# 18281818221/kalle-audio

Measured on AMD Instinct MI355X. Metric: audio-seconds/sec (node) DiT train step, 10s@12.5Hz x1024 latents, higher is better.
Workload: dtype bf16; 1 GPU; DiT train step (fwd+bwd+allreduce+Adam), 24 blocks D=1536 h=24, 10 s @ 12.5 Hz x 1024 latents (T=125+1 prepend), S=130 x 768 cross-attn cond; DiT shape chosen by this build (reference defines none); global_batch=256, per_gpu_batch=256, parallelism=dp1, objective=v, io_channels=1024, global_cond_type=prepend

## Files before the change

kalle_audio_amd/csrc/gemm2.hip:

```cpp
#include <stdio.h>
#include <stdlib.h>
#include <string.h>

#include <algorithm>
#include <functional>
#include <type_traits>
#include <utility>

#include "gemm_common.h"
#include "../../include/kalle_hip.h"

namespace {

constexpr int BK2 = 64;
#define GPTR(p) ((const __attribute__((address_space(1))) void*)(p))

__device__ __attribute__((aligned(64))) const unsigned kalle_zero_block[16] = {0, 0, 0, 0, 0, 0, 0, 0, 0, 0, 0, 0, 0, 0, 0, 0};

template <bool KM, int R, int NW>
struct Loader {
    static constexpr int PER_WAVE = (R / 8) / NW;
    const bf16_t* src[PER_WAVE];
    int64_t kstep;

    __device__ __forceinline__ void init(const bf16_t* X, int64_t ld, int Rtot, int r0, int k0, int wave, int lane,
                                         int glu_inner = 0, int glu_tn = 0) {
#pragma unroll
        for (int i = 0; i < PER_WAVE; ++i) {
            const int q = wave * PER_WAVE + i;
            if constexpr (!KM) {
                const int row = 8 * q + (lane >> 3);
                const int slot = lane & 7;
                const int c = slot ^ ((row >> 1) & 7);
                int gr = min(r0 + row, Rtot - 1);
                if (glu_inner > 0) {
                    const int wn_ = row >> 6, w_ = row & 63;
                    gr = (w_ >= 32 ? glu_inner : 0) + glu_tn * (R / 2) + wn_ * 32 + (w_ & 31);
                }
                src[i] = X + (int64_t)gr * ld + k0 + 8 * c;
            } else {
                constexpr int RB = 2 * R;
                constexpr int ROWS = 1024 / RB;
                const int pos = q * ROWS + (lane * 16) / RB;
                const int slot = ((lane * 16) % RB) / 16;
                const int c = slot ^ (2 * (pos & 7));
                const int krow = (pos & ~7) | ((pos & 7) ^ (((pos >> 3) & 1) << 2));
                const int gc = min(r0 + 8 * c, Rtot - 8);
                src[i] = X + (int64_t)(k0 + krow) * ld + gc;
            }
        }
        kstep = KM ? 64 * ld : 64;
    }
    __device__ __forceinline__ void issue(char* region, int wave) {
#pragma unroll
        for (int i = 0; i < PER_WAVE; ++i) {
            __builtin_amdgcn_global_load_lds(GPTR(src[i]), LDS_PTR(void, region + (wave * PER_WAVE + i) * 1024), 16, 0, 0);
            src[i] += kstep;
        }
    }
    __device__ __forceinline__ void issue_tail(char* region, int wave, int lane, int kvalid) {
#pragma unroll
        for (int i = 0; i < PER_WAVE; ++i) {
            const int q = wave * PER_WAVE + i;
            bool ok;
            if constexpr (!KM) {
                const int row = 8 * q + (lane >> 3);
                const int c = (lane & 7) ^ ((row >> 1) & 7);
                ok = 8 * c < kvalid;
            } else {
                constexpr int RB = 2 * R, ROWS = 1024 / RB;
                const int pos = q * ROWS + (lane * 16) / RB;
                const int krow = (pos & ~7) | ((pos & 7) ^ (((pos >> 3) & 1) << 2));
                ok = krow < kvalid;
            }
            const bf16_t* sp = ok ? src[i] : reinterpret_cast<const bf16_t*>(kalle_zero_block);
            __builtin_amdgcn_global_load_lds(GPTR(sp), LDS_PTR(void, region + (wave * PER_WAVE + i) * 1024), 16, 0, 0);
            src[i] += kstep;
        }
    }
    __device__ __forceinline__ void issue_at(char* region, int wave, int lane, int t, int tail_t, int kvalid) {
        if (t == tail_t) issue_tail(region, wave, lane, kvalid);
        else issue(region, wave);
    }
};

template <int OFF>
__device__ __forceinline__ i32x4 lds_b128(unsigned a) {
    i32x4 r;
    asm volatile("ds_read_b128 %0, %1 offset:%2" : "=v"(r) : "v"(a), "n"(OFF));
    return r;
}
__device__ __forceinline__ i32x2 lds_tr(unsigned a) {
    i32x2 r;
    asm volatile("ds_read_b64_tr_b16 %0, %1" : "=v"(r) : "v"(a));
    return r;
}

template <bool KM, int R>
struct Reader {
    unsigned b0[2], b1[2];
    __device__ __forceinline__ void init(int region_off, int rbase, int lane) {
#pragma unroll
        for (int s = 0; s < 2; ++s) {
            if constexpr (!KM) {
                const int row = rbase + (lane & 15);
                const int c = 4 * s + (lane >> 4);
                b0[s] = region_off + row * 128 + ((c ^ ((row >> 1) & 7)) << 4);
                b1[s] = 0;
            } else {
                constexpr int RB = 2 * R;
                const int g = lane >> 4, i = lane & 15;
                const int q = i >> 2, pp = i & 3;
                const int b = 4 * s + g;
                const int odd = b & 1;
                const int pos1 = 8 * b + (odd ? 4 : 0) + q;
                const int pos2 = 8 * b + (odd ? 0 : 4) + q;
                const int cl = (rbase >> 3) + (pp >> 1);
                const int hb = (pp & 1) * 8;
                b0[s] = region_off + pos1 * RB + ((cl ^ (2 * (pos1 & 7))) << 4) + hb;
                b1[s] = region_off + pos2 * RB + ((cl ^ (2 * (pos2 & 7))) << 4) + hb;
            }
        }
    }
    template <int S, int NTILE, int T0 = 0>
    __device__ __forceinline__ void read(unsigned so, i32x4 (&f)[NTILE]) const {
        if constexpr (!KM) {
            const unsigned a = b0[S] + so;
            f[0] = lds_b128<2048 * (T0 + 0)>(a);
            f[1] = lds_b128<2048 * (T0 + 1)>(a);
            f[2] = lds_b128<2048 * (T0 + 2)>(a);
            f[3] = lds_b128<2048 * (T0 + 3)>(a);
            if constexpr (NTILE == 8) {
                f[4] = lds_b128<2048 * (T0 + 4)>(a);
                f[5] = lds_b128<2048 * (T0 + 5)>(a);
                f[6] = lds_b128<2048 * (T0 + 6)>(a);
                f[7] = lds_b128<2048 * (T0 + 7)>(a);
            }
        } else {
            const unsigned a0 = b0[S] + so, a1 = b1[S] + so;
#pragma unroll
            for (int t = 0; t < NTILE; ++t) {
                const i32x2 lo = lds_tr(a0 ^ ((T0 + t) << 5));
                const i32x2 hi = lds_tr(a1 ^ ((T0 + t) << 5));
                f[t] = i32x4{lo[0], lo[1], hi[0], hi[1]};
            }
        }
    }
};

__device__ __forceinline__ void gemm_stamp(const GemmParams& p, int wave, int lane, int idx, int slot = -1) {
    if (p.stamps && (wave == 0 || wave == 7) && lane == 0)
        p.stamps[((int64_t)(slot < 0 ? (int)blockIdx.x : slot) * 2 + (wave ? 1 : 0)) * 8 + idx] = __builtin_amdgcn_s_memrealtime();
}

constexpr int EPI_DEPTH = 1;

struct NoHook { __device__ __forceinline__ void operator()() const {} };

__device__ __forceinline__ int pidx(int r, int c) { return r * 64 + (c ^ ((r & 1) << 2)); }

template <bool C_F32, int TM, int GLU = 0, typename Hook = NoHook>
__device__ __forceinline__ void wave_epilogue(const GemmParams& p, f32x4 (&acc)[TM][4], char* patch_base, int wave, int lane,
                                              int row0, int col0, Hook after_barrier = Hook{}, int stamp_slot = -1) {
    constexpr int DEPTH = EPI_DEPTH < TM ? EPI_DEPTH : TM;
    float* patch = reinterpret_cast<float*>(patch_base) + wave * (16 * 64);
    const int g = lane >> 4, li = lane & 15;
    const bool pre_res = C_F32 && GLU == 0 && !p.atomic && p.residual != nullptr;
    f32x4 rbuf[DEPTH][4];
    auto load_res = [&](int mt, f32x4 (&rv)[4]) {
#pragma unroll
        for (int i = 0; i < 4; ++i) {
            const int gm = row0 + 16 * mt + g + 4 * i, gn = col0 + 4 * li;
            rv[i] = f32x4{0.f, 0.f, 0.f, 0.f};
            if (gm < p.M && gn < p.N) rv[i] = *reinterpret_cast<const f32x4*>(p.residual + gemm_crow(p, gm) * p.ldr + gn);
        }
    };
    i32x4 hbuf[DEPTH][2][2];
    auto load_h = [&](int mt, i32x4 (&hv)[2][2]) {
        const int c8 = (lane & 7) * 8, j0 = col0 + c8;
#pragma unroll
        for (int half = 0; half < 2; ++half) {
            const int gm = row0 + 16 * mt + (lane >> 3) + 8 * half;
            hv[half][0] = i32x4{0, 0, 0, 0};
            hv[half][1] = i32x4{0, 0, 0, 0};
            if (gm < p.M && j0 < p.glu_inner) {
                const bf16_t* hp = static_cast<const bf16_t*>(p.glu_aux) + (int64_t)gm * 2 * p.glu_inner;
                hv[half][0] = *reinterpret_cast<const i32x4*>(hp + j0);
                hv[half][1] = *reinterpret_cast<const i32x4*>(hp + p.glu_inner + j0);
            }
        }
    };
    asm volatile("s_waitcnt lgkmcnt(0)" ::: "memory");
    __builtin_amdgcn_s_barrier();
    after_barrier();
    gemm_stamp(p, wave, lane, 3, stamp_slot);
#pragma unroll
    for (int d = 0; d < DEPTH; ++d) {
        if constexpr (GLU == 2) load_h(d, hbuf[d]);
        if (pre_res) load_res(d, rbuf[d]);
    }
    float sx[8], sg[8];
#pragma unroll
    for (int e = 0; e < 8; ++e) { sx[e] = 0.f; sg[e] = 0.f; }
    f32x4 bias4 = f32x4{0.f, 0.f, 0.f, 0.f}, bias8[2] = {f32x4{0.f, 0.f, 0.f, 0.f}, f32x4{0.f, 0.f, 0.f, 0.f}};
    float bx[8], bg[8];
#pragma unroll
    for (int e = 0; e < 8; ++e) { bx[e] = 0.f; bg[e] = 0.f; }
    if (p.bias) {
        if constexpr (GLU == 1) {
            const int j0 = col0 + (lane & 3) * 8;
            if (j0 < p.glu_inner) {
#pragma unroll
                for (int e = 0; e < 8; ++e) { bx[e] = p.bias[j0 + e]; bg[e] = p.bias[p.glu_inner + j0 + e]; }
            }
        } else if constexpr (GLU == 0) {
            if constexpr (C_F32) {
                if (!p.atomic && col0 + 4 * li < p.N) bias4 = *reinterpret_cast<const f32x4*>(p.bias + col0 + 4 * li);
            } else {
                const int gn = col0 + 8 * (lane & 7);
                if (gn < p.N) {
                    bias8[0] = *reinterpret_cast<const f32x4*>(p.bias + gn);
                    bias8[1] = *reinterpret_cast<const f32x4*>(p.bias + gn + 4);
                }
            }
        }
    }
#pragma unroll
    for (int mt = 0; mt < TM; ++mt) {
        const int slot = mt % DEPTH;
        f32x4 rcur[4];
        i32x4 hcur[2][2];
        if constexpr (GLU == 2) {
#pragma unroll
            for (int half = 0; half < 2; ++half) { hcur[half][0] = hbuf[slot][half][0]; hcur[half][1] = hbuf[slot][half][1]; }
            if (mt + DEPTH < TM) load_h(mt + DEPTH, hbuf[slot]);
        }
        if (pre_res) {
#pragma unroll
            for (int i = 0; i < 4; ++i) rcur[i] = rbuf[slot][i];
            if (mt + DEPTH < TM) load_res(mt + DEPTH, rbuf[slot]);
        }
#pragma unroll
        for (int nt = 0; nt < 4; ++nt)
#pragma unroll
            for (int r = 0; r < 4; ++r) patch[pidx(4 * g + r, 16 * nt + li)] = acc[mt][nt][r];
        asm volatile("s_waitcnt lgkmcnt(0)" ::: "memory");
        const int rbase = row0 + 16 * mt;
        if constexpr (GLU == 1) {
            const int r = lane >> 2, c8 = (lane & 3) * 8;
            const int gm = rbase + r, j0 = col0 + c8;
            if (gm < p.M && j0 < p.glu_inner) {
                float xv[8], gv[8];
#pragma unroll
                for (int e = 0; e < 8; ++e) { xv[e] = patch[pidx(r, c8 + e)]; gv[e] = patch[pidx(r, 32 + c8 + e)]; }
#pragma unroll
                for (int e = 0; e < 8; ++e) { xv[e] += bx[e]; gv[e] += bg[e]; }
                i32x4 hx, hg, av;
#pragma unroll
                for (int e = 0; e < 4; ++e) {
                    hx[e] = (int)pack_bf16x2(xv[2 * e], xv[2 * e + 1]);
                    hg[e] = (int)pack_bf16x2(gv[2 * e], gv[2 * e + 1]);
                    const float x0 = bf16lo((uint32_t)hx[e]), x1 = bf16hi((uint32_t)hx[e]);
                    const float g0 = bf16lo((uint32_t)hg[e]), g1 = bf16hi((uint32_t)hg[e]);
                    av[e] = (int)pack_bf16x2(x0 * siluf_(g0), x1 * siluf_(g1));
                }
                bf16_t* hp = reinterpret_cast<bf16_t*>(p.C) + (int64_t)gm * p.ldc;
                *reinterpret_cast<i32x4*>(hp + j0) = hx;
                *reinterpret_cast<i32x4*>(hp + p.glu_inner + j0) = hg;
                *reinterpret_cast<i32x4*>(static_cast<bf16_t*>(p.glu_aux) + (int64_t)gm * p.glu_inner + j0) = av;
            }
        } else if constexpr (GLU == 2) {
            const int c8 = (lane & 7) * 8, j0 = col0 + c8;
#pragma unroll
            for (int half = 0; half < 2; ++half) {
                const int r = (lane >> 3) + 8 * half;
                const int gm = rbase + r;
                if (gm < p.M && j0 < p.glu_inner) {
                    const i32x4 xv = hcur[half][0], gv = hcur[half][1];
                    i32x4 ox, og;
#pragma unroll
                    for (int e = 0; e < 4; ++e) {
                        const float x[2] = {bf16lo((uint32_t)xv[e]), bf16hi((uint32_t)xv[e])};
                        const float gg[2] = {bf16lo((uint32_t)gv[e]), bf16hi((uint32_t)gv[e])};
                        const float d[2] = {bf16_to_f32(f32_to_bf16(patch[pidx(r, c8 + 2 * e)] * p.alpha)),
                                            bf16_to_f32(f32_to_bf16(patch[pidx(r, c8 + 2 * e + 1)] * p.alpha))};
                        float dx[2], dg[2];
#pragma unroll
                        for (int q = 0; q < 2; ++q) {
                            const float sgm = sigmoidf_(gg[q]);
                            dx[q] = d[q] * gg[q] * sgm;
                            dg[q] = d[q] * x[q] * sgm * (1.f + gg[q] * (1.f - sgm));
                        }
                        ox[e] = (int)pack_bf16x2(dx[0], dx[1]);
                        og[e] = (int)pack_bf16x2(dg[0], dg[1]);
                        sx[2 * e] += bf16lo((uint32_t)ox[e]); sx[2 * e + 1] += bf16hi((uint32_t)ox[e]);
                        sg[2 * e] += bf16lo((uint32_t)og[e]); sg[2 * e + 1] += bf16hi((uint32_t)og[e]);
                    }
                    bf16_t* dp = reinterpret_cast<bf16_t*>(p.C) + (int64_t)gm * p.ldc;
                    *reinterpret_cast<i32x4*>(dp + j0) = ox;
                    *reinterpret_cast<i32x4*>(dp + p.glu_inner + j0) = og;
                }
            }
        } else if (p.atomic) {
            const int gn = col0 + lane;
#pragma unroll 4
            for (int r = 0; r < 16; ++r) {
                const int gm = rbase + r;
                if (gm < p.M && gn < p.N)
                    atomicAdd(reinterpret_cast<float*>(p.C) + (int64_t)gm * p.ldc + gn, patch[pidx(r, lane)] * p.alpha);
            }
        } else if constexpr (C_F32) {
#pragma unroll
            for (int i = 0; i < 4; ++i) {
                const int r = g + 4 * i;
                const int gm = rbase + r, gn = col0 + 4 * li;
                if (gm >= p.M || gn >= p.N) continue;
                const f32x4 pv = *reinterpret_cast<const f32x4*>(patch + pidx(r, 4 * li));
                float v[4] = {pv[0], pv[1], pv[2], pv[3]};
                const int64_t crow = gemm_crow(p, gm);
                gemm_epilogue4(p, gm, gn, crow, v, false, &bias4);
                if (pre_res) {
#pragma unroll
                    for (int j = 0; j < 4; ++j) v[j] += rcur[i][j];
                }
                float* cp = reinterpret_cast<float*>(p.C) + crow * p.ldc + gn;
                if (p.accumulate) {
                    const f32x4 c0 = *reinterpret_cast<const f32x4*>(cp);
#pragma unroll
                    for (int j = 0; j < 4; ++j) v[j] += c0[j];
                }
                *reinterpret_cast<f32x4*>(cp) = f32x4{v[0], v[1], v[2], v[3]};
            }
        } else {
#pragma unroll
            for (int half = 0; half < 2; ++half) {
                const int r = (lane >> 3) + 8 * half;
                const int gm = rbase + r, gn = col0 + 8 * (lane & 7);
                if (gm >= p.M || gn >= p.N) continue;
                const f32x4 p0 = *reinterpret_cast<const f32x4*>(patch + pidx(r, 8 * (lane & 7)));
                const f32x4 p1 = *reinterpret_cast<const f32x4*>(patch + pidx(r, 8 * (lane & 7) + 4));
                float v0[4] = {p0[0], p0[1], p0[2], p0[3]}, v1[4] = {p1[0], p1[1], p1[2], p1[3]};
                const int64_t crow = gemm_crow(p, gm);
                gemm_epilogue4(p, gm, gn, crow, v0, true, &bias8[0]);
                gemm_epilogue4(p, gm, gn + 4, crow, v1, true, &bias8[1]);
                i32x4 o;
                o[0] = (int)pack_bf16x2(v0[0], v0[1]);
                o[1] = (int)pack_bf16x2(v0[2], v0[3]);
                o[2] = (int)pack_bf16x2(v1[0], v1[1]);
                o[3] = (int)pack_bf16x2(v1[2], v1[3]);
                *reinterpret_cast<i32x4*>(reinterpret_cast<bf16_t*>(p.C) + crow * p.ldc + gn) = o;
            }
        }
        asm volatile("s_waitcnt lgkmcnt(0)" ::: "memory");
    }
    if constexpr (GLU == 2) {
        if (p.glu_dbias) {
#pragma unroll
            for (int e = 0; e < 8; ++e) {
#pragma unroll
                for (int o = 8; o < 64; o <<= 1) { sx[e] += __shfl_xor(sx[e], o, 64); sg[e] += __shfl_xor(sg[e], o, 64); }
            }
            const int j0 = col0 + (lane & 7) * 8;
            if (lane < 8 && j0 < p.glu_inner) {
#pragma unroll
                for (int e = 0; e < 8; ++e) {
                    atomicAdd(p.glu_dbias + j0 + e, sx[e]);
                    atomicAdd(p.glu_dbias + p.glu_inner + j0 + e, sg[e]);
                }
            }
        }
    }
    if (p.stamps) {
        gemm_stamp(p, wave, lane, 4, stamp_slot);
        asm volatile("s_waitcnt vmcnt(0)" ::: "memory");
        gemm_stamp(p, wave, lane, 5, stamp_slot);
    }
}

#define MFMA16(FA, FB)                                                                                         \
    _Pragma("unroll") for (int mt = 0; mt < 4; ++mt) _Pragma("unroll") for (int nt = 0; nt < 4; ++nt)          \
        acc[mt][nt] = __builtin_amdgcn_mfma_f32_16x16x32_bf16(__builtin_bit_cast(bf16x8, FA[mt]),              \
                                                              __builtin_bit_cast(bf16x8, FB[nt]), acc[mt][nt], 0, 0, 0)

template <bool A_KM, bool B_KM, bool C_F32, int WM, int WN, int TM, int GLU = 0, int NS = 3>
__global__ __launch_bounds__(WM * WN * 64, 2) void gemm2_kernel(GemmParams p) {
    static_assert(TM == 4, "wave tile is 64 x 64");
    constexpr int TN = 4;
    constexpr int NW = WM * WN;
    constexpr int BM = WM * TM * 16, BN = WN * TN * 16;
    constexpr int A_BYTES = BM * 128, B_BYTES = BN * 128, STAGE = A_BYTES + B_BYTES;
    extern __shared__ __attribute__((aligned(16))) char smem[];
    const unsigned lds0 = (unsigned)(size_t)LDS_PTR(char, smem);

    const int tid = threadIdx.x, lane = tid & 63;
    const int wave = __builtin_amdgcn_readfirstlane(tid >> 6);
    const int wm = wave / WN, wn = wave % WN;

    int tm, tn;
    gemm_tile_coords(blockIdx.x, gridDim.x, p.tiles_m, p.tiles_n, p.group_m, tm, tn);
    const int m0 = tm * BM, n0 = tn * BN;

    const int nk_all = (p.K + BK2 - 1) / BK2;
    const int kt0 = blockIdx.y * p.ktiles_per_split;
    const int nk = min(p.ktiles_per_split, nk_all - kt0);
    const int kvalid = p.K % BK2;
    const int tail_t = kvalid ? nk_all - 1 - kt0 : -1;

    f32x4 acc[TM][TN];
#pragma unroll
    for (int i = 0; i < TM; ++i)
#pragma unroll
        for (int j = 0; j < TN; ++j) acc[i][j] = f32x4{0.f, 0.f, 0.f, 0.f};

    Loader<A_KM, BM, NW> la;
    Loader<B_KM, BN, NW> lb;
    la.init(p.A, p.lda, p.M, m0, kt0 * BK2, wave, lane);
    lb.init(p.B, p.ldb, p.N, n0, kt0 * BK2, wave, lane, GLU == 1 ? p.glu_inner : 0, tn);
    const int arow = wm * TM * 16, bcol = wn * TN * 16;
    Reader<A_KM, BM> ra;
    Reader<B_KM, BN> rb;
    ra.init(lds0, arow, lane);
    rb.init(lds0 + A_BYTES, bcol, lane);

    {
    constexpr int PT = Loader<A_KM, BM, NW>::PER_WAVE + Loader<B_KM, BN, NW>::PER_WAVE;
    static_assert((NS - 2) * PT <= 63, "vmcnt is a 6-bit counter");
    {
        const int pre = nk < NS ? nk : NS;
#pragma unroll
        for (int t = 0; t < NS; ++t) {
            if (t < pre) {
                la.issue_at(smem + t * STAGE, wave, lane, t, tail_t, kvalid);
                lb.issue_at(smem + t * STAGE + A_BYTES, wave, lane, t, tail_t, kvalid);
            }
        }
        constexpr int PRE_KEEP = (NS - 1) * PT <= 63 ? NS - 1 : NS - 2;
        const int keep = pre - 1 < PRE_KEEP ? pre - 1 : PRE_KEEP;
        auto wait_keep = [&](auto self, auto c) {
            constexpr int C = decltype(c)::value;
            if (keep == C) asm volatile("s_waitcnt vmcnt(%0)" ::"n"(C * PT) : "memory");
            if constexpr (C > 0) self(self, std::integral_constant<int, C - 1>{});
        };
        wait_keep(wait_keep, std::integral_constant<int, PRE_KEEP>{});
    }
    __builtin_amdgcn_s_barrier();
    __builtin_amdgcn_sched_barrier(0);

    i32x4 fa0[4], fb0[4], fa1[4], fb1[4];
    ra.template read<0, 4>(0, fa0);
    rb.template read<0, 4>(0, fb0);

    unsigned so_cur = 0, so_nxt = STAGE;
    int kt = 0;

    auto iteration = [&](auto issue_c, auto next_c, auto keep_c) {
        constexpr bool ISSUE = decltype(issue_c)::value, NEXT = decltype(next_c)::value;
        constexpr int KEEP = decltype(keep_c)::value;
        asm volatile("s_waitcnt lgkmcnt(0)" ::: "memory");
        __builtin_amdgcn_sched_barrier(0);
        ra.template read<1, 4>(so_cur, fa1);
        rb.template read<1, 4>(so_cur, fb1);
        __builtin_amdgcn_sched_barrier(0);
        MFMA16(fa0, fb0);
        __builtin_amdgcn_sched_barrier(0);
        asm volatile("s_waitcnt vmcnt(%0) lgkmcnt(0)" ::"n"(KEEP * PT) : "memory");
        __builtin_amdgcn_s_barrier();
        __builtin_amdgcn_sched_barrier(0);
        if (wave >= NW / 2) {
            MFMA16(fa1, fb1);
            __builtin_amdgcn_sched_barrier(0);
        }
        if constexpr (ISSUE) {
            la.issue_at(smem + so_cur, wave, lane, kt + NS, tail_t, kvalid);
            lb.issue_at(smem + so_cur + A_BYTES, wave, lane, kt + NS, tail_t, kvalid);
        }
        if constexpr (NEXT) {
            ra.template read<0, 4>(so_nxt, fa0);
            rb.template read<0, 4>(so_nxt, fb0);
        }
        __builtin_amdgcn_sched_barrier(0);
        if (wave < NW / 2) {
            MFMA16(fa1, fb1);
            __builtin_amdgcn_sched_barrier(0);
        }
        so_cur = so_nxt;
        so_nxt = so_nxt + STAGE >= NS * STAGE ? 0 : so_nxt + STAGE;
    };
    using T_ = std::true_type;
    using F_ = std::false_type;
#pragma unroll 1
    for (; kt + NS < nk; ++kt) iteration(T_{}, T_{}, std::integral_constant<int, NS - 2>{});
    auto tail = [&](auto self, auto r) {
        constexpr int R = decltype(r)::value;
        if (nk - 1 - kt == R) { iteration(F_{}, T_{}, std::integral_constant<int, R - 1>{}); ++kt; }
        if constexpr (R > 1) self(self, std::integral_constant<int, R - 1>{});
    };
    tail(tail, std::integral_constant<int, NS - 1>{});
    iteration(F_{}, F_{}, std::integral_constant<int, 0>{});
    }

    if constexpr (C_F32) {
        if (p.slab_stride) {
            GemmParams q = p;
            q.C = static_cast<float*>(p.C) + (int64_t)blockIdx.y * p.slab_stride;
            wave_epilogue<C_F32, TM>(q, acc, smem, wave, lane, m0 + arow, n0 + bcol);
            return;
        }
    }
    wave_epilogue<C_F32, TM, GLU>(p, acc, smem, wave, lane, m0 + arow, GLU == 1 ? tn * (BN / 2) + wn * 32 : n0 + bcol);
}


template <bool B_KM, bool C_F32, int WM, int WN, int GLU, int NS>
__global__ __launch_bounds__(WM * WN * 128, 1) void gemm2_ks2_kernel(GemmParams p) {
    static_assert(!B_KM || WN >= 2, "a k-major operand tile needs >= 128 columns (16 swizzle slots per k-row)");
    constexpr int TM = 4, TN = 4;
    constexpr int NWT = WM * WN, NW = 2 * NWT;
    constexpr int BM = WM * 64, BN = WN * 64;
    constexpr int A_BYTES = BM * 128, B_BYTES = BN * 128, STAGE = A_BYTES + B_BYTES;
    constexpr int RED_OFF = 32768;
    static_assert(RED_OFF + NWT * 16384 <= NS * STAGE, "partial-sum exchange must fit into the ring");
    extern __shared__ __attribute__((aligned(16))) char smem[];
    const unsigned lds0 = (unsigned)(size_t)LDS_PTR(char, smem);

    const int tid = threadIdx.x, lane = tid & 63;
    const int wave = __builtin_amdgcn_readfirstlane(tid >> 6);
    const int kg = wave / NWT, wt = wave % NWT;
    const int wm = wt / WN, wn = wt % WN;

// ... 180 lines not shown
__device__ __forceinline__ int sched_resolve(int xcd, int raw, int first_round, int ntiles) {
    const int id = xcd + 8 * (first_round + raw);
    return id < ntiles ? id : ntiles;
}
__device__ __forceinline__ void sched_leave(int* sched, int nwg) {
    if (atomicAdd(sched + 8 * SCHED_LINE, 1) == nwg - 1) {
#pragma unroll
        for (int i = 0; i < 9; ++i) atomicExch(sched + i * SCHED_LINE, 0);
    }
}

template <bool A_KM, bool B_KM, bool C_F32, int GLU, bool XCD_RASTER, bool PERSIST>
__device__ __forceinline__ void gemm3_tiles(const GemmParams& p, int tile0, int tstride, int tile_end, int ntiles_raster, int kt0,
                                            int nk) {
    const int kvalid = p.K % BK2;
    const int tail_t = kvalid ? (p.K + BK2 - 1) / BK2 - 1 - kt0 : -1;
    constexpr int WN = 4, TM = 8, NW = 8;
    constexpr int BM = 256, BN = 256;
    constexpr int A_BYTES = BM * 128, B_BYTES = BN * 128, STAGE = A_BYTES + B_BYTES;
    extern __shared__ __attribute__((aligned(16))) char smem[];
    const unsigned lds0 = (unsigned)(size_t)LDS_PTR(char, smem);

    const int tid = threadIdx.x, lane = tid & 63;
    const int wave = __builtin_amdgcn_readfirstlane(tid >> 6);
    const int wm = wave / WN, wn = wave % WN;
    const int arow = wm * 128, bcol = wn * 64;
    Loader<A_KM, BM, NW> la;
    Loader<B_KM, BN, NW> lb;
    Reader<A_KM, BM> ra;
    Reader<B_KM, BN> rb;
    ra.init(lds0, arow, lane);
    rb.init(lds0 + A_BYTES, bcol, lane);
    const bool late = wave >= NW / 2;
    if (late) __builtin_amdgcn_s_setprio(1);

    auto coords = [&](int tile, int& tm, int& tn) {
        if constexpr (XCD_RASTER) gemm_tile_coords(tile, ntiles_raster, p.tiles_m, p.tiles_n, p.group_m, tm, tn);
        else gemm_tile_coords_plain(tile, p.tiles_m, p.tiles_n, p.group_m, tm, tn);
    };
    auto init_loaders = [&](int tm, int tn, int kt_first) {
        la.init(p.A, p.lda, p.M, tm * BM, (kt0 + kt_first) * BK2, wave, lane);
        lb.init(p.B, p.ldb, p.N, tn * BN, (kt0 + kt_first) * BK2, wave, lane, GLU == 1 ? p.glu_inner : 0, tn);
    };
    bool prefetched = false;
    unsigned s0 = 0;

    int* const sched = PERSIST && p.sched_set > 0 ? &kalle_gemm_sched[p.sched_set - 1][0] : nullptr;
    int next_tile = tile_end;
    int drawn = 0;
    if constexpr (PERSIST) {
        if (sched && tid == 0) drawn = sched_issue(sched, blockIdx.x & 7);
    }
    volatile int* const mailbox = reinterpret_cast<volatile int*>(smem + 2 * STAGE);
    for (int tile = tile0; tile < tile_end; tile = next_tile) {
        int tm, tn;
        coords(tile, tm, tn);
        const int m0 = tm * BM, n0 = tn * BN;
        next_tile = PERSIST ? tile + tstride : tile_end;
        bool has_next = PERSIST && next_tile < tile_end;
        gemm_stamp(p, wave, lane, 0, tile);
        f32x4 acc[TM][4];
#pragma unroll
        for (int i = 0; i < TM; ++i)
#pragma unroll
            for (int j = 0; j < 4; ++j) acc[i][j] = f32x4{0.f, 0.f, 0.f, 0.f};

        if (!prefetched) {
            init_loaders(tm, tn, 0);
            la.issue_at(smem, wave, lane, 0, tail_t, kvalid);
            lb.issue_at(smem + A_BYTES, wave, lane, 0, tail_t, kvalid);
            s0 = 0;
            if (nk > 1) {
                la.issue_at(smem + STAGE, wave, lane, 1, tail_t, kvalid);
                lb.issue_at(smem + STAGE + A_BYTES, wave, lane, 1, tail_t, kvalid);
                asm volatile("s_waitcnt vmcnt(8)" ::: "memory");
            } else {
                asm volatile("s_waitcnt vmcnt(0)" ::: "memory");
            }
        } else if constexpr (PERSIST) {
            init_loaders(tm, tn, nk > 1 ? 2 : 1);
            asm volatile("s_waitcnt vmcnt(0)" ::: "memory");
        }
        if constexpr (PERSIST) {
            if (sched && tid == 0) {
                *mailbox = sched_resolve(blockIdx.x & 7, drawn, tstride >> 3, tile_end);
                asm volatile("s_waitcnt lgkmcnt(0)" ::: "memory");
            }
        }
        __builtin_amdgcn_s_barrier();
        __builtin_amdgcn_sched_barrier(0);
        if constexpr (PERSIST) {
            if (sched) {
                next_tile = __builtin_amdgcn_readfirstlane(*mailbox);
                has_next = next_tile < tile_end;
            }
        }
        gemm_stamp(p, wave, lane, 1, tile);

        i32x4 fa[8], fb[4];
        unsigned so_cur = s0;
        int kt = 0;
        ra.template read<0, 8>(so_cur, fa);
        rb.template read<0, 4>(so_cur, fb);

        auto iteration = [&](auto issue_c, auto next_c) {
            constexpr bool ISSUE = decltype(issue_c)::value, NEXT = decltype(next_c)::value;
            asm volatile("s_waitcnt lgkmcnt(0)" ::: "memory");
            __builtin_amdgcn_sched_barrier(0);
            MFMA32(fa, fb);
            __builtin_amdgcn_sched_barrier(0);
            ra.template read<1, 8>(so_cur, fa);
            rb.template read<1, 4>(so_cur, fb);
            asm volatile("s_waitcnt lgkmcnt(0)" ::: "memory");
            __builtin_amdgcn_sched_barrier(0);
            if (!late) {
                MFMA32(fa, fb);
                __builtin_amdgcn_sched_barrier(0);
            }
            asm volatile("s_waitcnt vmcnt(0)" ::: "memory");
            __builtin_amdgcn_s_barrier();
            __builtin_amdgcn_sched_barrier(0);
            if (late) {
                MFMA32(fa, fb);
                __builtin_amdgcn_sched_barrier(0);
            }
            if constexpr (ISSUE) {
                la.issue_at(smem + so_cur, wave, lane, kt + 2, tail_t, kvalid);
                lb.issue_at(smem + so_cur + A_BYTES, wave, lane, kt + 2, tail_t, kvalid);
            }
            so_cur ^= STAGE;
            if constexpr (NEXT) {
                ra.template read<0, 8>(so_cur, fa);
                rb.template read<0, 4>(so_cur, fb);
            }
            __builtin_amdgcn_sched_barrier(0);
        };
        auto last_iteration = [&]() {
            asm volatile("s_waitcnt lgkmcnt(0)" ::: "memory");
            __builtin_amdgcn_sched_barrier(0);
            MFMA32(fa, fb);
            __builtin_amdgcn_sched_barrier(0);
            ra.template read<1, 8>(so_cur, fa);
            rb.template read<1, 4>(so_cur, fb);
            asm volatile("s_waitcnt lgkmcnt(0)" ::: "memory");
            __builtin_amdgcn_sched_barrier(0);
            MFMA32(fa, fb);
            __builtin_amdgcn_sched_barrier(0);
        };
        using T_ = std::true_type;
        using F_ = std::false_type;
#pragma unroll 1
        for (; kt + 2 < nk; ++kt) iteration(T_{}, T_{});
        if (kt + 1 < nk) { iteration(F_{}, T_{}); ++kt; }
        if constexpr (!PERSIST || GLU == 2) iteration(F_{}, F_{});
        else last_iteration();
        gemm_stamp(p, wave, lane, 2, tile);

        const unsigned s_last = so_cur;
        auto hook = [&]() {
            if constexpr (!PERSIST) return;
            if (has_next) {
                int ntm, ntn;
                coords(next_tile, ntm, ntn);
                init_loaders(ntm, ntn, 0);
                la.issue_at(smem + (s_last ^ STAGE), wave, lane, 0, tail_t, kvalid);
                lb.issue_at(smem + (s_last ^ STAGE) + A_BYTES, wave, lane, 0, tail_t, kvalid);
                if (nk > 1) {
                    la.issue_at(smem + s_last, wave, lane, 1, tail_t, kvalid);
                    lb.issue_at(smem + s_last + A_BYTES, wave, lane, 1, tail_t, kvalid);
                }
                if (sched && tid == 0) drawn = sched_issue(sched, blockIdx.x & 7);
            }
        };
        wave_epilogue<C_F32, TM, GLU>(p, acc, smem + 2 * STAGE, wave, lane, m0 + arow, GLU == 1 ? tn * 128 + wn * 32 : n0 + bcol,
                                      hook, tile);
        prefetched = has_next;
        s0 = s_last ^ STAGE;
        if constexpr (!PERSIST) break;
    }
}

template <bool A_KM, bool B_KM, bool C_F32, int GLU = 0>
__global__ __launch_bounds__(512, 2) void gemm3_kernel(GemmParams p) {
    const int nk_all = (p.K + BK2 - 1) / BK2;
    const int ntiles = p.tiles_m * p.tiles_n;
    if constexpr (A_KM) {
        if (p.mix_na >= 0) {
            const int na = p.mix_na, sa = p.mix_sa;
            int bid = blockIdx.x, tile, slice, per;
            if (bid < na * sa) { tile = bid % na; slice = bid / na; per = (nk_all + sa - 1) / sa; }
            else { bid -= na * sa; const int nb = ntiles - na; tile = na + bid % nb; slice = bid / nb; per = (nk_all + sa) / (sa + 1); }
            const int kt0 = slice * per, nk = min(per, nk_all - kt0);
            if (nk <= 0) return;
            gemm3_tiles<A_KM, B_KM, C_F32, GLU, true, false>(p, tile, 0, tile + 1, ntiles, kt0, nk);
        } else {
            const int kt0 = blockIdx.y * p.ktiles_per_split;
            gemm3_tiles<A_KM, B_KM, C_F32, GLU, true, false>(p, blockIdx.x, 0, blockIdx.x + 1, ntiles, kt0,
                                                             min(p.ktiles_per_split, nk_all - kt0));
        }
    } else {
        gemm3_tiles<A_KM, B_KM, C_F32, GLU, true, true>(p, blockIdx.x, gridDim.x, ntiles, ntiles, 0, nk_all);
        if (p.sched_set > 0 && threadIdx.x == 0) sched_leave(&kalle_gemm_sched[p.sched_set - 1][0], gridDim.x);
    }
}

struct GroupProblem {
    const bf16_t* A;
    const bf16_t* B;
    float* C;
    int64_t lda, ldb, ldc;
    int M, N, K;
    int tiles_m, tiles_n, group_m;
    int unsplit, splits;
    int r1_start, r2_start;
};
struct GroupParams {
    int nprob, r2_base;
    int overwrite;
    GroupProblem pr[KALLE_MAX_GROUP];
};

__global__ __launch_bounds__(256) void gemm3_group_zero_kernel(GroupParams gp) {
    int pi = 0, base = 0;
    const int bid = blockIdx.x >> 2, band = blockIdx.x & 3;
    for (;;) {
        const int nb = gp.pr[pi].tiles_m * gp.pr[pi].tiles_n - gp.pr[pi].unsplit;
        if (bid < base + nb || pi + 1 >= gp.nprob) break;
        base += nb;
        ++pi;
    }
    const GroupProblem& q = gp.pr[pi];
    int tm, tn;
    gemm_tile_coords_plain(q.unsplit + bid - base, q.tiles_m, q.tiles_n, q.group_m, tm, tn);
    const int r0 = tm * 256 + band * 64, c0 = tn * 256;
    for (int i = threadIdx.x; i < 64 * 64; i += 256) {
        const int r = r0 + i / 64, c = c0 + (i & 63) * 4;
        if (r < q.M && c < q.N) *reinterpret_cast<f32x4*>(q.C + (int64_t)r * q.ldc + c) = f32x4{0.f, 0.f, 0.f, 0.f};
    }
}

__global__ __launch_bounds__(512, 2) void gemm3_wgrad_group_kernel(GroupParams gp) {
    const bool whole = (int)blockIdx.x < gp.r2_base;
    const int bid = whole ? xcd_contiguous(blockIdx.x, gp.r2_base)
                          : gp.r2_base + xcd_contiguous(blockIdx.x - gp.r2_base, gridDim.x - gp.r2_base);
    int pi = 0, tile, slice = 0;
    if (whole) {
        while (pi + 1 < gp.nprob && bid >= gp.pr[pi + 1].r1_start) ++pi;
        tile = bid - gp.pr[pi].r1_start;
    } else {
        while (pi + 1 < gp.nprob && bid >= gp.pr[pi + 1].r2_start) ++pi;
        const int local = bid - gp.pr[pi].r2_start, nb = gp.pr[pi].tiles_m * gp.pr[pi].tiles_n - gp.pr[pi].unsplit;
        tile = gp.pr[pi].unsplit + local % nb;
        slice = local / nb;
    }
    const GroupProblem& q = gp.pr[pi];
    GemmParams p{};
    p.A = q.A; p.B = q.B; p.C = q.C;
    p.lda = q.lda; p.ldb = q.ldb; p.ldc = q.ldc;
    p.M = q.M; p.N = q.N; p.K = q.K;
    p.alpha = 1.f;
    p.rows_per_batch = 1;
    p.accumulate = gp.overwrite ? 0 : 1;
    p.atomic = whole ? 0 : 1;
    const int ntiles = q.tiles_m * q.tiles_n, nk_all = (q.K + BK2 - 1) / BK2;
    p.tiles_m = q.tiles_m; p.tiles_n = q.tiles_n; p.group_m = q.group_m;
    int kt0 = 0, nk = nk_all;
    if (!whole) {
        const int per = (nk_all + q.splits - 1) / q.splits;
        kt0 = slice * per;
        nk = min(per, nk_all - kt0);
        if (nk <= 0) return;
    }
    gemm3_tiles<true, true, true, 0, false, false>(p, tile, 0, tile + 1, ntiles, kt0, nk);
}

template <bool A_KM, bool B_KM, bool C_F32, int GLU = 0>
int launch3(const GemmParams& p, hipStream_t st) {
    constexpr int lds = GEMM3_LDS;
    static std::atomic<uint64_t> lds_ok{0};
    kalle_allow_lds(reinterpret_cast<const void*>(gemm3_kernel<A_KM, B_KM, C_F32, GLU>), lds, lds_ok);
    dim3 grid(p.tiles_m * p.tiles_n, p.splits), block(512);
    if (p.mix_na >= 0) {
        const int ntiles = p.tiles_m * p.tiles_n;
        grid = dim3(p.mix_na * p.mix_sa + (ntiles - p.mix_na) * (p.mix_sa + 1), 1);
    } else if (!A_KM) {
        if (p.splits != 1) return KALLE_ERR_UNSUPPORTED;
        const int cus = kalle_cu_count();
        if ((int)grid.x > cus) {
            GemmParams q = p;
            grid.x = cus;
            static std::atomic<unsigned> next_set{0};
            hipStreamCaptureStatus cap = hipStreamCaptureStatusNone;
            const bool capturing = hipStreamIsCapturing(st, &cap) == hipSuccess && cap != hipStreamCaptureStatusNone;
            q.sched_set = !capturing ? 1 + (int)(next_set.fetch_add(1, std::memory_order_relaxed) % SCHED_SETS) : 0;
            KALLE_LAUNCH((gemm3_kernel<A_KM, B_KM, C_F32, GLU>), grid, block, lds, st, q);
            return kalle_check_launch();
        }
    }
    KALLE_LAUNCH((gemm3_kernel<A_KM, B_KM, C_F32, GLU>), grid, block, lds, st, p);
    return kalle_check_launch();
}

int launch3_layout(const GemmParams& p, bool a_km, bool b_km, bool f32, hipStream_t st) {
    if (!a_km && !b_km) return f32 ? launch3<false, false, true>(p, st) : launch3<false, false, false>(p, st);
    if (!a_km && b_km) return f32 ? launch3<false, true, true>(p, st) : launch3<false, true, false>(p, st);
    if (a_km && b_km) return launch3<true, true, true>(p, st);
    return KALLE_ERR_UNSUPPORTED;
// ... 525 lines not shown
```

Baseline: 11700 audio-seconds/sec.

## Pack SwiGLU epilogue patch to bf16 with DPP swizzle and double-buffered halves

Splits the GEMM epilogue into a plain path and a SwiGLU path. The SwiGLU forward and backward epilogues now convert accumulators to bf16 in registers, swap pairs across lanes with DPP and byte permutes, and write a half-size packed LDS patch with a bank-conflict-free swizzle that is verified by static asserts. Each row tile is read back as one 128-bit load per half. The patch is double-buffered so the next tile's pack-and-write overlaps the current tile's global stores. This cuts LDS traffic and scalar conversions in the epilogue. In exchange it adds more complex indexing, and persistent GLU kernels no longer use the last_iteration path.

```diff
diff --git a/kalle_audio_amd/csrc/gemm2.hip b/kalle_audio_amd/csrc/gemm2.hip
--- a/kalle_audio_amd/csrc/gemm2.hip
+++ b/kalle_audio_amd/csrc/gemm2.hip
@@ -159,22 +159,80 @@
 
 __device__ __forceinline__ int pidx(int r, int c) { return r * 64 + (c ^ ((r & 1) << 2)); }
 
-template <bool C_F32, int TM, int GLU = 0, typename Hook = NoHook>
-__device__ __forceinline__ void wave_epilogue(const GemmParams& p, f32x4 (&acc)[TM][4], char* patch_base, int wave, int lane,
-                                              int row0, int col0, Hook after_barrier = Hook{}, int stamp_slot = -1) {
+constexpr int PP_HALF = 16 * 32;
+constexpr int ppidx(int r, int ch) { return r * 32 + ((ch ^ (((r >> 1) & 3) << 1)) << 2); }
+constexpr int pp_write_idx(int lane, int nt, int j) {
+    const int g = lane >> 4, li = lane & 15;
+    const int r = 4 * g + 2 * (li & 1) + j, c = 16 * nt + (li & ~1);
+    return ppidx(r, c >> 3) + ((c >> 1) & 3);
+}
+constexpr int pp_read_idx(int lane, int half) { return ppidx((lane >> 3) + 8 * half, lane & 7); }
+constexpr int pp_read_idx_glu1(int lane, int gate) { return ppidx(lane >> 2, (lane & 3) + 4 * gate); }
+
+constexpr int b128_group(int lane) {
+    const int l = lane & 31;
+    const bool a = l < 4 || (l >= 12 && l < 16) || (l >= 20 && l < 28);
+    return 2 * (lane >> 5) + (a ? 0 : 1);
+}
+template <typename F>
+constexpr bool b128_conflict_free(F idx) {
+    for (int grp = 0; grp < 4; ++grp) {
+        unsigned long long used = 0;
+        for (int lane = 0; lane < 64; ++lane) {
+            if (b128_group(lane) != grp) continue;
+            for (int d = 0; d < 4; ++d) {
+                const unsigned long long bit = 1ull << ((idx(lane) + d) & 63);
+                if (used & bit) return false;
+                used |= bit;
+            }
+        }
+    }
+    return true;
+}
+constexpr bool pp_writes_conflict_free() {
+    for (int nt = 0; nt < 4; ++nt)
+        for (int j = 0; j < 2; ++j)
+            for (int grp = 0; grp < 2; ++grp) {
+                unsigned used = 0;
+                for (int lane = 32 * grp; lane < 32 * grp + 32; ++lane) {
+                    const unsigned bit = 1u << (pp_write_idx(lane, nt, j) & 31);
+                    if (used & bit) return false;
+                    used |= bit;
+                }
+            }
+    return true;
+}
+struct PpRead0 { constexpr int operator()(int lane) const { return pp_read_idx(lane, 0); } };
+struct PpRead1 { constexpr int operator()(int lane) const { return pp_read_idx(lane, 1); } };
+struct PpReadX { constexpr int operator()(int lane) const { return pp_read_idx_glu1(lane, 0); } };
+struct PpReadG { constexpr int operator()(int lane) const { return pp_read_idx_glu1(lane, 1); } };
+static_assert(pp_writes_conflict_free(), "packed patch: ds_write_b32 bank conflict");
+static_assert(b128_conflict_free(PpRead0{}) && b128_conflict_free(PpRead1{}), "packed patch: row read bank conflict");
+static_assert(b128_conflict_free(PpReadX{}) && b128_conflict_free(PpReadG{}), "packed patch: SwiGLU forward read bank conflict");
+
+constexpr bool pp_shortcuts_hold() {
+    for (int lane = 0; lane < 64; ++lane) {
+        for (int nt = 0; nt < 4; ++nt)
+            for (int j = 0; j < 2; ++j)
+                if (pp_write_idx(lane, nt, j) != (pp_write_idx(lane, 0, 0) ^ (8 * nt)) + 32 * j) return false;
+        if (pp_read_idx(lane, 1) != pp_read_idx(lane, 0) + 8 * 32) return false;
+        if (pp_read_idx_glu1(lane, 1) != (pp_read_idx_glu1(lane, 0) ^ 16)) return false;
+    }
+    return true;
+}
+static_assert(pp_shortcuts_hold(), "packed patch: index shortcuts");
+
+constexpr unsigned PERM_LO_EVEN = 0x05040100u, PERM_HI_EVEN = 0x07060302u, PERM_LO_ODD = 0x01000504u, PERM_HI_ODD = 0x03020706u;
+
+template <int TM, int GLU, typename Hook>
+__device__ __forceinline__ void wave_epilogue_glu(const GemmParams& p, f32x4 (&acc)[TM][4], char* patch_base, int wave, int lane,
+                                                   int row0, int col0, Hook after_barrier, int stamp_slot) {
+    static_assert(GLU == 1 || GLU == 2, "the plain epilogues keep the fp32 patch");
     constexpr int DEPTH = EPI_DEPTH < TM ? EPI_DEPTH : TM;
-    float* patch = reinterpret_cast<float*>(patch_base) + wave * (16 * 64);
+    asm volatile("" : "+v"(lane));
+    uint32_t* patch = reinterpret_cast<uint32_t*>(patch_base) + wave * (2 * PP_HALF);
     const int g = lane >> 4, li = lane & 15;
-    const bool pre_res = C_F32 && GLU == 0 && !p.atomic && p.residual != nullptr;
-    f32x4 rbuf[DEPTH][4];
-    auto load_res = [&](int mt, f32x4 (&rv)[4]) {
-#pragma unroll
-        for (int i = 0; i < 4; ++i) {
-            const int gm = row0 + 16 * mt + g + 4 * i, gn = col0 + 4 * li;
-            rv[i] = f32x4{0.f, 0.f, 0.f, 0.f};
-            if (gm < p.M && gn < p.N) rv[i] = *reinterpret_cast<const f32x4*>(p.residual + gemm_crow(p, gm) * p.ldr + gn);
-        }
-    };
+    const bool odd = li & 1;
     i32x4 hbuf[DEPTH][2][2];
     auto load_h = [&](int mt, i32x4 (&hv)[2][2]) {
         const int c8 = (lane & 7) * 8, j0 = col0 + c8;
@@ -197,93 +255,86 @@
 #pragma unroll
     for (int d = 0; d < DEPTH; ++d) {
         if constexpr (GLU == 2) load_h(d, hbuf[d]);
-        if (pre_res) load_res(d, rbuf[d]);
     }
     float sx[8], sg[8];
 #pragma unroll
     for (int e = 0; e < 8; ++e) { sx[e] = 0.f; sg[e] = 0.f; }
-    f32x4 bias4 = f32x4{0.f, 0.f, 0.f, 0.f}, bias8[2] = {f32x4{0.f, 0.f, 0.f, 0.f}, f32x4{0.f, 0.f, 0.f, 0.f}};
-    float bx[8], bg[8];
-#pragma unroll
-    for (int e = 0; e < 8; ++e) { bx[e] = 0.f; bg[e] = 0.f; }
+    float bcol[4] = {0.f, 0.f, 0.f, 0.f};
     if (p.bias) {
-        if constexpr (GLU == 1) {
-            const int j0 = col0 + (lane & 3) * 8;
-            if (j0 < p.glu_inner) {
-#pragma unroll
-                for (int e = 0; e < 8; ++e) { bx[e] = p.bias[j0 + e]; bg[e] = p.bias[p.glu_inner + j0 + e]; }
-            }
-        } else if constexpr (GLU == 0) {
-            if constexpr (C_F32) {
-                if (!p.atomic && col0 + 4 * li < p.N) bias4 = *reinterpret_cast<const f32x4*>(p.bias + col0 + 4 * li);
-            } else {
-                const int gn = col0 + 8 * (lane & 7);
-                if (gn < p.N) {
-                    bias8[0] = *reinterpret_cast<const f32x4*>(p.bias + gn);
-                    bias8[1] = *reinterpret_cast<const f32x4*>(p.bias + gn + 4);
-                }
-            }
-        }
-    }
+#pragma unroll
+        for (int nt = 0; nt < 4; ++nt) {
+            if constexpr (GLU == 1) {
+                const int j = col0 + 16 * (nt & 1) + li;
+                if (j < p.glu_inner) bcol[nt] = p.bias[(nt >= 2 ? p.glu_inner : 0) + j];
+            }
+        }
+    }
+    const uint32_t sel_lo = odd ? PERM_LO_ODD : PERM_LO_EVEN, sel_hi = odd ? PERM_HI_ODD : PERM_HI_EVEN;
+    const int widx = pp_write_idx(lane, 0, 0);
+    const int ridx = GLU == 1 ? pp_read_idx_glu1(lane, 0) : pp_read_idx(lane, 0);
+
+    auto pack_and_write = [&](int mt) {
+        uint32_t* half = patch + (mt & 1) * PP_HALF;
+#pragma unroll
+        for (int nt = 0; nt < 4; ++nt) {
+            float v[4];
+#pragma unroll
+            for (int r = 0; r < 4; ++r) {
+                if constexpr (GLU == 1) v[r] = acc[mt][nt][r] + bcol[nt];
+                else v[r] = acc[mt][nt][r] * p.alpha;
+            }
+            const uint32_t p01 = pack_bf16x2(v[0], v[1]), p23 = pack_bf16x2(v[2], v[3]);
+            const uint32_t keep = odd ? p23 : p01, give = odd ? p01 : p23;
+            const uint32_t got = (uint32_t)__builtin_amdgcn_update_dpp(0, (int)give, 0xB1, 0xF, 0xF, true);
+            half[(widx ^ (8 * nt))] = __builtin_amdgcn_perm(got, keep, sel_lo);
+            half[(widx ^ (8 * nt)) + 32] = __builtin_amdgcn_perm(got, keep, sel_hi);
+        }
+    };
+    pack_and_write(0);
 #pragma unroll
     for (int mt = 0; mt < TM; ++mt) {
         const int slot = mt % DEPTH;
-        f32x4 rcur[4];
         i32x4 hcur[2][2];
         if constexpr (GLU == 2) {
 #pragma unroll
             for (int half = 0; half < 2; ++half) { hcur[half][0] = hbuf[slot][half][0]; hcur[half][1] = hbuf[slot][half][1]; }
             if (mt + DEPTH < TM) load_h(mt + DEPTH, hbuf[slot]);
         }
-        if (pre_res) {
-#pragma unroll
-            for (int i = 0; i < 4; ++i) rcur[i] = rbuf[slot][i];
-            if (mt + DEPTH < TM) load_res(mt + DEPTH, rbuf[slot]);
-        }
-#pragma unroll
-        for (int nt = 0; nt < 4; ++nt)
-#pragma unroll
-            for (int r = 0; r < 4; ++r) patch[pidx(4 * g + r, 16 * nt + li)] = acc[mt][nt][r];
         asm volatile("s_waitcnt lgkmcnt(0)" ::: "memory");
+        const uint32_t* half = patch + (mt & 1) * PP_HALF;
+        const i32x4 q0 = *reinterpret_cast<const i32x4*>(half + ridx);
+        const i32x4 q1 = *reinterpret_cast<const i32x4*>(half + (GLU == 1 ? ridx ^ 16 : ridx + 8 * 32));
+        if (mt + 1 < TM) pack_and_write(mt + 1);
         const int rbase = row0 + 16 * mt;
         if constexpr (GLU == 1) {
             const int r = lane >> 2, c8 = (lane & 3) * 8;
             const int gm = rbase + r, j0 = col0 + c8;
             if (gm < p.M && j0 < p.glu_inner) {
-                float xv[8], gv[8];
-#pragma unroll
-                for (int e = 0; e < 8; ++e) { xv[e] = patch[pidx(r, c8 + e)]; gv[e] = patch[pidx(r, 32 + c8 + e)]; }
-#pragma unroll
-                for (int e = 0; e < 8; ++e) { xv[e] += bx[e]; gv[e] += bg[e]; }
-                i32x4 hx, hg, av;
+                i32x4 av;
 #pragma unroll
                 for (int e = 0; e < 4; ++e) {
-                    hx[e] = (int)pack_bf16x2(xv[2 * e], xv[2 * e + 1]);
-                    hg[e] = (int)pack_bf16x2(gv[2 * e], gv[2 * e + 1]);
-                    const float x0 = bf16lo((uint32_t)hx[e]), x1 = bf16hi((uint32_t)hx[e]);
-                    const float g0 = bf16lo((uint32_t)hg[e]), g1 = bf16hi((uint32_t)hg[e]);
+                    const float x0 = bf16lo((uint32_t)q0[e]), x1 = bf16hi((uint32_t)q0[e]);
+                    const float g0 = bf16lo((uint32_t)q1[e]), g1 = bf16hi((uint32_t)q1[e]);
                     av[e] = (int)pack_bf16x2(x0 * siluf_(g0), x1 * siluf_(g1));
                 }
                 bf16_t* hp = reinterpret_cast<bf16_t*>(p.C) + (int64_t)gm * p.ldc;
-                *reinterpret_cast<i32x4*>(hp + j0) = hx;
-                *reinterpret_cast<i32x4*>(hp + p.glu_inner + j0) = hg;
+                *reinterpret_cast<i32x4*>(hp + j0) = q0;
+                *reinterpret_cast<i32x4*>(hp + p.glu_inner + j0) = q1;
                 *reinterpret_cast<i32x4*>(static_cast<bf16_t*>(p.glu_aux) + (int64_t)gm * p.glu_inner + j0) = av;
             }
-        } else if constexpr (GLU == 2) {
+        } else {
             const int c8 = (lane & 7) * 8, j0 = col0 + c8;
 #pragma unroll
-            for (int half = 0; half < 2; ++half) {
-                const int r = (lane >> 3) + 8 * half;
-                const int gm = rbase + r;
+            for (int half_ = 0; half_ < 2; ++half_) {
+                const int gm = rbase + (lane >> 3) + 8 * half_;
                 if (gm < p.M && j0 < p.glu_inner) {
-                    const i32x4 xv = hcur[half][0], gv = hcur[half][1];
+                    const i32x4 xv = hcur[half_][0], gv = hcur[half_][1], dv = half_ ? q1 : q0;
                     i32x4 ox, og;
 #pragma unroll
                     for (int e = 0; e < 4; ++e) {
                         const float x[2] = {bf16lo((uint32_t)xv[e]), bf16hi((uint32_t)xv[e])};
                         const float gg[2] = {bf16lo((uint32_t)gv[e]), bf16hi((uint32_t)gv[e])};
-                        const float d[2] = {bf16_to_f32(f32_to_bf16(patch[pidx(r, c8 + 2 * e)] * p.alpha)),
-                                            bf16_to_f32(f32_to_bf16(patch[pidx(r, c8 + 2 * e + 1)] * p.alpha))};
+                        const float d[2] = {bf16lo((uint32_t)dv[e]), bf16hi((uint32_t)dv[e])};
                         float dx[2], dg[2];
 #pragma unroll
                         for (int q = 0; q < 2; ++q) {
@@ -301,7 +352,84 @@
                     *reinterpret_cast<i32x4*>(dp + p.glu_inner + j0) = og;
                 }
             }
-        } else if (p.atomic) {
+        }
+    }
+    if constexpr (GLU == 2) {
+        if (p.glu_dbias) {
+#pragma unroll
+            for (int e = 0; e < 8; ++e) {
+#pragma unroll
+                for (int o = 8; o < 64; o <<= 1) { sx[e] += __shfl_xor(sx[e], o, 64); sg[e] += __shfl_xor(sg[e], o, 64); }
+            }
+            const int j0 = col0 + (lane & 7) * 8;
+            if (lane < 8 && j0 < p.glu_inner) {
+#pragma unroll
+                for (int e = 0; e < 8; ++e) {
+                    atomicAdd(p.glu_dbias + j0 + e, sx[e]);
+                    atomicAdd(p.glu_dbias + p.glu_inner + j0 + e, sg[e]);
+                }
+            }
+        }
+    }
+    if (p.stamps) {
+        gemm_stamp(p, wave, lane, 4, stamp_slot);
+        asm volatile("s_waitcnt vmcnt(0)" ::: "memory");
+        gemm_stamp(p, wave, lane, 5, stamp_slot);
+    }
+}
+
+template <bool C_F32, int TM, typename Hook>
+__device__ __forceinline__ void wave_epilogue_plain(const GemmParams& p, f32x4 (&acc)[TM][4], char* patch_base, int wave, int lane,
+                                                  int row0, int col0, Hook after_barrier, int stamp_slot) {
+    constexpr int DEPTH = EPI_DEPTH < TM ? EPI_DEPTH : TM;
+    float* patch = reinterpret_cast<float*>(patch_base) + wave * (16 * 64);
+    const int g = lane >> 4, li = lane & 15;
+    const bool pre_res = C_F32 && !p.atomic && p.residual != nullptr;
+    f32x4 rbuf[DEPTH][4];
+    auto load_res = [&](int mt, f32x4 (&rv)[4]) {
+#pragma unroll
+        for (int i = 0; i < 4; ++i) {
+            const int gm = row0 + 16 * mt + g + 4 * i, gn = col0 + 4 * li;
+            rv[i] = f32x4{0.f, 0.f, 0.f, 0.f};
+            if (gm < p.M && gn < p.N) rv[i] = *reinterpret_cast<const f32x4*>(p.residual + gemm_crow(p, gm) * p.ldr + gn);
+        }
+    };
+    asm volatile("s_waitcnt lgkmcnt(0)" ::: "memory");
+    __builtin_amdgcn_s_barrier();
+    after_barrier();
+    gemm_stamp(p, wave, lane, 3, stamp_slot);
+#pragma unroll
+    for (int d = 0; d < DEPTH; ++d) {
+        if (pre_res) load_res(d, rbuf[d]);
+    }
+    f32x4 bias4 = f32x4{0.f, 0.f, 0.f, 0.f}, bias8[2] = {f32x4{0.f, 0.f, 0.f, 0.f}, f32x4{0.f, 0.f, 0.f, 0.f}};
+    if (p.bias) {
+        if constexpr (C_F32) {
+            if (!p.atomic && col0 + 4 * li < p.N) bias4 = *reinterpret_cast<const f32x4*>(p.bias + col0 + 4 * li);
+        } else {
+            const int gn = col0 + 8 * (lane & 7);
+            if (gn < p.N) {
+                bias8[0] = *reinterpret_cast<const f32x4*>(p.bias + gn);
+                bias8[1] = *reinterpret_cast<const f32x4*>(p.bias + gn + 4);
+            }
+        }
+    }
+#pragma unroll
+    for (int mt = 0; mt < TM; ++mt) {
+        const int slot = mt % DEPTH;
+        f32x4 rcur[4];
+        if (pre_res) {
+#pragma unroll
+            for (int i = 0; i < 4; ++i) rcur[i] = rbuf[slot][i];
+            if (mt + DEPTH < TM) load_res(mt + DEPTH, rbuf[slot]);
+        }
+#pragma unroll
+        for (int nt = 0; nt < 4; ++nt)
+#pragma unroll
+            for (int r = 0; r < 4; ++r) patch[pidx(4 * g + r, 16 * nt + li)] = acc[mt][nt][r];
+        asm volatile("s_waitcnt lgkmcnt(0)" ::: "memory");
+        const int rbase = row0 + 16 * mt;
+        if (p.atomic) {
             const int gn = col0 + lane;
 #pragma unroll 4
             for (int r = 0; r < 16; ++r) {
@@ -353,28 +481,19 @@
         }
         asm volatile("s_waitcnt lgkmcnt(0)" ::: "memory");
     }
-    if constexpr (GLU == 2) {
-        if (p.glu_dbias) {
-#pragma unroll
-            for (int e = 0; e < 8; ++e) {
-#pragma unroll
-                for (int o = 8; o < 64; o <<= 1) { sx[e] += __shfl_xor(sx[e], o, 64); sg[e] += __shfl_xor(sg[e], o, 64); }
-            }
-            const int j0 = col0 + (lane & 7) * 8;
-            if (lane < 8 && j0 < p.glu_inner) {
-#pragma unroll
-                for (int e = 0; e < 8; ++e) {
-                    atomicAdd(p.glu_dbias + j0 + e, sx[e]);
-                    atomicAdd(p.glu_dbias + p.glu_inner + j0 + e, sg[e]);
-                }
-            }
-        }
-    }
     if (p.stamps) {
         gemm_stamp(p, wave, lane, 4, stamp_slot);
         asm volatile("s_waitcnt vmcnt(0)" ::: "memory");
         gemm_stamp(p, wave, lane, 5, stamp_slot);
     }
+}
+
+template <bool C_F32, int TM, int GLU = 0, typename Hook = NoHook>
+__device__ __forceinline__ void wave_epilogue(const GemmParams& p, f32x4 (&acc)[TM][4], char* patch_base, int wave, int lane,
+                                              int row0, int col0, Hook after_barrier = Hook{}, int stamp_slot = -1) {
+    static_assert(GLU == 0 || !C_F32, "the fused SwiGLU epilogues write bf16");
+    if constexpr (GLU == 0) wave_epilogue_plain<C_F32, TM>(p, acc, patch_base, wave, lane, row0, col0, after_barrier, stamp_slot);
+    else wave_epilogue_glu<TM, GLU>(p, acc, patch_base, wave, lane, row0, col0, after_barrier, stamp_slot);
 }
 
 #define MFMA16(FA, FB)                                                                                         \
@@ -861,7 +980,7 @@
 #pragma unroll 1
         for (; kt + 2 < nk; ++kt) iteration(T_{}, T_{});
         if (kt + 1 < nk) { iteration(F_{}, T_{}); ++kt; }
-        if constexpr (!PERSIST || GLU == 2) iteration(F_{}, F_{});
+        if constexpr (!PERSIST || GLU != 0) iteration(F_{}, F_{});
         else last_iteration();
         gemm_stamp(p, wave, lane, 2, tile);
 
```

After: 11780 audio-seconds/sec (median of 6 runs). About the same (+0.7%).
